# taaha-khan/2023-CompaCT-Image-Compression

Measured on AMD Instinct MI355X. Metric: MPixels/s encode+decode, 12-bit 512x512 CT batch, bytes-exact, higher is better.
Workload: dtype u16

## Files before the change

2023-compact-image-compression_amd/csrc/deflate_kernels.hip:

```cpp
#include <hip/hip_runtime.h>
#include <cstring>
#include <algorithm>

#include "cct_internal.h"
#include "../../include/compact_hip.h"

namespace cct {
namespace {

constexpr int MIN_MATCH = 3, MAX_MATCH = 258, WSIZE = 32768;
constexpr int MIN_LOOKAHEAD = MAX_MATCH + MIN_MATCH + 1;
constexpr int MAX_DIST = WSIZE - MIN_LOOKAHEAD;
constexpr int TOO_FAR = 4096;
constexpr int BLOCK_SYMS = 16383;
constexpr int BLOCK_SYMS_ML9 = 32767;
constexpr int L_CODES = 286, D_CODES = 30, BL_CODES = 19, HEAP_SIZE = 2 * L_CODES + 1;
constexpr int END_BLOCK = 256, MAX_BITS = 15, MAX_BL_BITS = 7;
constexpr uint32_t Z_FILTERED = 1, Z_HUFFMAN_ONLY = 2, Z_RLE = 3, Z_FIXED = 4;
__host__ __device__ __forceinline__ bool short_pass(uint32_t strategy) { return strategy == Z_HUFFMAN_ONLY || strategy == Z_RLE; }

__constant__ uint8_t c_extra_lbits[29] = {0,0,0,0,0,0,0,0,1,1,1,1,2,2,2,2,3,3,3,3,4,4,4,4,5,5,5,5,0};
__constant__ uint8_t c_extra_dbits[30] = {0,0,0,0,1,1,2,2,3,3,4,4,5,5,6,6,7,7,8,8,9,9,10,10,11,11,12,12,13,13};
__constant__ uint8_t c_extra_blbits[19] = {0,0,0,0,0,0,0,0,0,0,0,0,0,0,0,0,2,3,7};
__constant__ uint8_t c_bl_order[19] = {16,17,18,0,8,7,9,6,10,5,11,4,12,3,13,2,14,1,15};
__constant__ uint8_t c_length_code[256];
__constant__ uint16_t c_base_length[29];
__constant__ uint8_t c_dist_code[512];
__constant__ uint16_t c_base_dist[30];
__constant__ uint16_t c_static_lcode[288];
__constant__ uint8_t c_static_llen[288];
__constant__ uint16_t c_static_dcode[30];

template <int HB>
__device__ __forceinline__ uint32_t hash3(uint32_t b0, uint32_t b1, uint32_t b2)
{
	constexpr int SH = (HB + 2) / 3;
	return ((b0 << (2 * SH)) ^ (b1 << SH) ^ b2) & ((1u << HB) - 1u);
}

__device__ __forceinline__ int d_code(uint32_t dist) { return dist < 256 ? c_dist_code[dist] : c_dist_code[256 + (dist >> 7)]; }

struct MatchRec { uint16_t len_full, len_quarter, dist_full, dist_quarter; };
constexpr uint32_t GEN_MAX = 16383;
__device__ __forceinline__ uint2 pack_match(uint32_t len_full, uint32_t len_quarter, uint32_t dist_full, uint32_t dist_quarter, uint32_t gen)
{
	return make_uint2((len_full | ((gen & 127u) << 9)) | ((len_quarter | ((gen >> 7) << 9)) << 16), dist_full | (dist_quarter << 16));
}
__device__ __forceinline__ MatchRec checked_match(MatchRec r, uint32_t gen, uint32_t rw, uint32_t p, uint32_t L)
{
	const uint32_t tag = (uint32_t)(r.len_full >> 9) | ((uint32_t)(r.len_quarter >> 9) << 7);
	const uint32_t lookahead = L - min(p, L);
	const uint32_t max_len = lookahead < (uint32_t)MAX_MATCH ? lookahead : (uint32_t)MAX_MATCH;
	const bool maximal = (rw >> 15) && (rw & 0x7FFFu) >= max_len && p + 2 < L;
	MatchRec o;
	const bool ok = tag == gen;
// ... 58 lines not shown
#ifdef CCT_SORT_PROBE
	const bool compact = false;
#else
	const bool compact = HB == 15 && a.pos_mask != 0xFFFFFFFFu;
#endif
	const uint32_t dmax = (uint32_t)a.in_stride - 4u;
	auto fetch = [&](uint32_t tile_base, uint32_t (&ra)[E], uint32_t (&rb)[E]) {
		if (FIRST) {
#pragma unroll
			for (int d = 0; d < ND; d++) ra[d] = *reinterpret_cast<const uint32_t *>(in + min(tile_base + 256u * d + 4u * (uint32_t)lane, dmax));
			ra[ND] = *reinterpret_cast<const uint32_t *>(in + min(tile_base + 256u * ND, dmax));
#pragma unroll
			for (int e = 0; e < E; e++) rb[e] = compact ? a.run_len[base + min(tile_base + (uint32_t)(e * 64 + lane), last)] : 0u;
		} else {
#pragma unroll
			for (int e = 0; e < E; e++) {
				const uint64_t r = rec_src[min(tile_base + (uint32_t)(e * 64 + lane), last)];
				ra[e] = (uint32_t)r; rb[e] = (uint32_t)(r >> 32);
			}
		}
	};
	auto finish = [&](uint32_t tile_base, const uint32_t (&ra)[E], const uint32_t (&rb)[E], uint32_t (&h)[E], uint32_t (&p)[E]) {
#pragma unroll
		for (int e = 0; e < E; e++) {
			const uint32_t idx = tile_base + (uint32_t)(e * 64 + lane);
			if (FIRST) {
				const int la = (e & 3) * 16 + (lane >> 2);
				const uint32_t da = (uint32_t)__builtin_amdgcn_ds_bpermute(la << 2, (int)ra[e >> 2]);
				uint32_t db = (uint32_t)__builtin_amdgcn_ds_bpermute(((la + 1) & 63) << 2, (int)ra[e >> 2]);
				if ((e & 3) == 3) {
					const uint32_t nxt = (e >> 2) + 1 < ND ? (uint32_t)__builtin_amdgcn_readfirstlane((int)ra[(e >> 2) + 1 < ND ? (e >> 2) + 1 : 0]) : ra[ND];
					if (la == 63) db = nxt;
				}
				const uint32_t sh = (uint32_t)lane & 3u;
				const uint32_t w = __builtin_amdgcn_alignbyte(db, da, sh);
				const uint32_t b0 = w & 255u, b1 = (w >> 8) & 255u, b2 = (w >> 16) & 255u;
				h[e] = hash3<HB>(b0, b1, b2); p[e] = idx;
				if (compact) {
					const uint32_t b4 = (db >> (8u * sh)) & 255u;
					const uint32_t f16 = (b0 == b1 && b1 == b2) ? rb[e] : ((w >> 24) | (b4 << 8));
					h[e] |= (f16 << 15) | ((b0 >> 7) << 31); p[e] |= (b1 << 22) | (((b0 >> 5) & 3u) << 30);
				}
			}
			else { h[e] = rb[e]; p[e] = ra[e]; }
			if (idx >= npos) { h[e] = 0; p[e] = idx; }
		}
	};
	uint32_t hn[E], pn[E];
	{
		uint32_t ra[E], rb[E];
		fetch((uint32_t)(wave * 64 * E), ra, rb);
		finish((uint32_t)(wave * 64 * E), ra, rb, hn, pn);
	}
	for (uint32_t t0 = 0; t0 < npos; t0 += 1024 * E) {
		uint32_t h[E], p[E], rk[E], ra[E], rb[E];
		const uint32_t idx0 = t0 + (uint32_t)(wave * 64 * E + lane);
#pragma unroll
		for (int e = 0; e < E; e++) { h[e] = hn[e]; p[e] = pn[e]; }
		const uint32_t next_base = t0 + (uint32_t)(1024 * E + wave * 64 * E);
		fetch(next_base, ra, rb);
		for (int k = lane; k < NB; k += 64) wcnt[wave][k] = 0;
#pragma unroll
		for (int e = 0; e < E; e++) {
			const bool valid = idx0 + e * 64 < npos;
			const uint32_t d = FIRST ? (h[e] & 255u) : ((h[e] & HMASK) >> 8);
			uint64_t same = __ballot(valid);
#pragma unroll
			for (int b = 0; b < BITS; b++) {
				const bool bit = (d >> b) & 1u;
				const uint64_t bal = __ballot(bit);
				same &= bit ? bal : ~bal;
			}
			const uint32_t rank = (uint32_t)__popcll(same & lt_mask);
			uint32_t before = 0;
			if (valid) {
				before = wcnt[wave][d];
				if (rank == 0) wcnt[wave][d] = before + (uint32_t)__popcll(same);
			}
			rk[e] = before + rank;
		}
		lds_barrier();
		if (tid < NB) {
			uint32_t c[16], run = offs[tid];
#pragma unroll
			for (int w = 0; w < 16; w++) c[w] = wcnt[w][tid];
#pragma unroll
			for (int w = 0; w < 16; w++) { wcnt[w][tid] = run; run += c[w]; }
			offs[tid] = run;
		}
		lds_barrier();
#pragma unroll
		for (int e = 0; e < E; e++) asm volatile("" : "+v"(ra[e]), "+v"(rb[e]) :: "memory");
		finish(next_base, ra, rb, hn, pn);
#pragma unroll
		for (int e = 0; e < E; e++) {
			if (idx0 + e * 64 < npos) {
				const uint32_t d = FIRST ? (h[e] & 255u) : ((h[e] & HMASK) >> 8);
				const uint32_t dst = wcnt[wave][d] + rk[e];
				rec_dst[dst] = (uint64_t)p[e] | ((uint64_t)h[e] << 32);
			}
		}
	}
}

constexpr int LIGHT_STEPS = 12;

__device__ __forceinline__ bool xcd_slice(int n, int &s, uint32_t &part, uint32_t &nparts)
{
	const uint32_t lin = blockIdx.x + gridDim.x * blockIdx.y;
	const uint32_t c = lin & 7u, k = lin >> 3;
	nparts = gridDim.x;
	s = (int)(8u * (k / nparts) + c);
	part = k % nparts;
	return s < n;
}

__device__ __forceinline__ uint32_t nil_candidate(uint32_t p, uint32_t lookahead)
{
	return (lookahead < (uint32_t)MIN_LOOKAHEAD && p >= 32506u + 32768u && (p - 32506u) % 32768u == 0) ? p - 32506u : 0xFFFFFFFFu;
}

constexpr int RUNLEN_OUT = 2048 - 264;

template <bool SORT, int HB>
__global__ void __launch_bounds__(256) dfl_run_len_kernel(DeflateArgs a)
{
	constexpr int NH = 256 + (1 << (HB - 8));
	__shared__ uint32_t wtot[4];
	__shared__ uint32_t hist[SORT ? NH : 1];
	if (SORT) for (int t = threadIdx.x; t < NH; t += 256) hist[t] = 0;
	__syncthreads();
	const int s = blockIdx.y;
	const uint32_t L = a.in_sizes[s];
	const uint8_t *in = a.in + (size_t)s * a.in_stride;
	uint16_t *rl = a.run_len + (size_t)s * a.in_stride;
	const int lane = threadIdx.x & 63, wave = threadIdx.x >> 6;
	const uint32_t nchunks = (L + RUNLEN_OUT - 1) / RUNLEN_OUT;
	for (uint32_t c = blockIdx.x; c < nchunks; c += gridDim.x) {
		const uint32_t c0 = c * RUNLEN_OUT;
		const uint32_t g = c0 + threadIdx.x * 8;
		uint8_t b[12];
		if (g + 12 <= L && g >= 1) {
			uint64_t w;
			__builtin_memcpy(&w, in + g, 8);
#pragma unroll
			for (int k = 0; k < 8; k++) b[k + 1] = (uint8_t)(w >> (8 * k));
			b[0] = in[g - 1];
			uint32_t w2; __builtin_memcpy(&w2, in + g + 8, 4);
			b[9] = (uint8_t)w2; b[10] = (uint8_t)(w2 >> 8); b[11] = (uint8_t)(w2 >> 16);
		} else {
#pragma unroll
			for (int k = 0; k < 12; k++) { const int64_t y = (int64_t)g - 1 + k; b[k] = (y >= 0 && y < (int64_t)L) ? in[y] : 0; }
		}
		if (SORT) {
// ... 509 lines not shown
{
	len = 2; dist = 0;
	if (p >= npos || prev_len >= lazy) return;
	match_of(checked_match(mr[p], gen, rl[p], p, npos + 2), p, npos, prev_len, lazy, good, minl, len, dist);
}

__global__ void __launch_bounds__(256) dfl_rec_kernel(DeflateArgs a)
{
	const int s = blockIdx.y;
	const uint32_t L = a.in_sizes[s];
	const size_t base = (size_t)s * a.in_stride;
	const uint32_t npos = L >= MIN_MATCH ? L - 2 : 0;
	const MatchRec *mr = reinterpret_cast<const MatchRec *>(a.mr) + base;
	const uint16_t *rl = a.run_len + base;
	const uint32_t nblk64 = (L + 63) / 64;
	const int lane = threadIdx.x & 63;
	const uint32_t gen = *a.gen;
	const int lazy = (int)a.max_lazy, good = (int)a.good, minl = (int)a.min_len;
	const uint32_t lastp = npos ? npos - 1 : 0;
	const uint32_t wb_step = gridDim.x * (blockDim.x >> 6);
	struct Req { MatchRec m0, m1; uint32_t w0, w1; };
	auto request = [&](uint32_t wb) {
		const uint32_t p = wb * 64 + lane, pa = min(p, lastp), pb = min(p + 1, lastp);
		return Req{mr[pa], mr[pb], rl[pa], rl[pb]};
	};
	const uint32_t wb0 = blockIdx.x * (blockDim.x >> 6) + (threadIdx.x >> 6);
	Req nx = request(wb0);
	for (uint32_t wb = wb0; wb < nblk64; wb += wb_step) {
		const uint32_t p = wb * 64 + lane;
		const uint32_t blk_end = wb * 64 + 64;
		uint32_t rec = 0, nxt = blk_end, cnt = 0;
		const uint32_t pa = min(p, lastp), pb = min(p + 1, lastp);
		const Req cq = nx;
		nx = request(wb + wb_step);
		const MatchRec r0 = checked_match(cq.m0, gen, cq.w0, pa, L), r1 = checked_match(cq.m1, gen, cq.w1, pb, L);
		if (p < L) {
			int len, dist;
			match_of(r0, p, npos, 2, lazy, good, minl, len, dist);
			if (len < MIN_MATCH) { rec = 0; nxt = p + 1; cnt = 1; }
			else {
				uint32_t k = 0;
				for (;;) {
					int l2, d2;
					if (k == 0) match_of(r1, p + 1, npos, len, lazy, good, minl, l2, d2);
					else match_at(mr, rl, gen, p + k + 1, npos, len, lazy, good, minl, l2, d2);
					if (l2 > len) { len = l2; dist = d2; k++; } else break;
				}
				rec = k | ((uint32_t)len << 8) | ((uint32_t)dist << 17);
				nxt = p + k + (uint32_t)len;
				cnt = k + 1;
			}
		}
		a.rec32[base + p] = rec;
#pragma unroll
		for (int r = 0; r < 6; r++) {
			const bool inside = nxt < blk_end;
			const int j = inside ? (int)(nxt - wb * 64) : lane;
			const uint32_t n2 = __shfl(nxt, j), c2 = __shfl(cnt, j);
			if (inside) { nxt = n2; cnt += c2; }
		}
		a.exit_pos[base + p] = (nxt - blk_end) | (cnt << 16);
	}
}

__global__ void __launch_bounds__(256) dfl_rle_rec_kernel(DeflateArgs a)
{
	const int s = blockIdx.y;
	const uint32_t L = a.in_sizes[s];
	const size_t base = (size_t)s * a.in_stride;
	const uint16_t *rl = a.run_len + base;
	const uint32_t nblk64 = (L + 63) / 64;
	const int lane = threadIdx.x & 63;
	const uint32_t lastp = L ? L - 1 : 0;
	const uint32_t wb_step = gridDim.x * (blockDim.x >> 6);
	const uint32_t wb0 = blockIdx.x * (blockDim.x >> 6) + (threadIdx.x >> 6);
	uint32_t nx = rl[min(wb0 * 64 + lane, lastp)];
	for (uint32_t wb = wb0; wb < nblk64; wb += wb_step) {
		const uint32_t p = wb * 64 + lane;
		const uint32_t blk_end = wb * 64 + 64;
		const uint32_t rw = nx;
		nx = rl[min((wb + wb_step) * 64 + lane, lastp)];
		const uint32_t rw0 = (uint32_t)__shfl((int)rw, 0);
		const bool prev_eq = p >= 2 ? (rw >> 15) != 0 : (p == 1 && (rw0 & 0x7FFFu) >= 2u);
		const uint32_t run = rw & 0x7FFFu;
		uint32_t rec = 0, nxt = blk_end, cnt = 0;
		if (p < L) {
			const bool m = prev_eq && run >= (uint32_t)MIN_MATCH;
			rec = m ? (run << 8) | (1u << 17) : 0u;
			nxt = p + (m ? run : 1u);
			cnt = 1;
		}
		a.rec32[base + p] = rec;
#pragma unroll
		for (int r = 0; r < 6; r++) {
			const bool inside = nxt < blk_end;
			const int j = inside ? (int)(nxt - wb * 64) : lane;
			const uint32_t n2 = __shfl(nxt, j), c2 = __shfl(cnt, j);
			if (inside) { nxt = n2; cnt += c2; }
		}
		a.exit_pos[base + p] = (nxt - blk_end) | (cnt << 16);
	}
}

template <uint32_t BS>
__global__ void __launch_bounds__(256) dfl_huff_symbols_kernel(DeflateArgs a)
{
	const int s = blockIdx.y;
	const uint32_t L = a.in_sizes[s];
	const size_t base = (size_t)s * a.in_stride;
	const uint32_t *in4 = reinterpret_cast<const uint32_t *>(a.in + base);
	uint4 *sym4 = reinterpret_cast<uint4 *>(a.sym + base);
	uint32_t *bend = a.blk_end + (size_t)s * a.max_blocks, *btop = a.blk_top + (size_t)s * a.max_blocks;
	if (blockIdx.x == 0 && threadIdx.x == 0) a.total_syms[s] = L;
	const uint32_t nq = (L + 3) / 4;
	for (uint32_t q = blockIdx.x * blockDim.x + threadIdx.x; q < nq; q += gridDim.x * blockDim.x) {
		const uint32_t w = in4[q], p0 = 4 * q;
		uint32_t v[4];
#pragma unroll
		for (int k = 0; k < 4; k++) {
			const uint32_t p = p0 + (uint32_t)k;
			v[k] = p < L ? (w >> (8 * k)) & 255u : 0u;
			if (p < L && p % BS == BS - 1) { bend[p / BS] = p + 1; btop[p / BS] = p; }
		}
		sym4[q] = make_uint4(v[0], v[1], v[2], v[3]);
	}
}

#ifndef CCT_WALK_T
#define CCT_WALK_T 256
#endif
constexpr int WALK_T = CCT_WALK_T;
__global__ void __launch_bounds__(WALK_T) dfl_walk_kernel(DeflateArgs a, int n)
{
	__shared__ uint32_t s_land[WALK_T];
	__shared__ uint32_t s_wsum[WALK_T / 64];
	const int s = blockIdx.x;
	(void)n;
	const uint32_t L = a.in_sizes[s];
	const size_t base = (size_t)s * a.in_stride;
	const size_t bbase = (size_t)s * (a.in_stride / 64);
	const uint32_t *exit_rec = a.exit_pos + base;
	const int tid = threadIdx.x, lane = tid & 63, wave = tid >> 6;
	const uint32_t seg = (((L + WALK_T - 1) / WALK_T) + 63) & ~63u;
	const uint32_t seg_end = min(L, (uint32_t)(tid + 1) * seg);
	uint32_t start = min(L, (uint32_t)tid * seg), land = start, cnt = 0;
// ... 646 lines not shown
	for (int q = 0; q < nb; q++) {
		TreeScratch &S = S4[q];
		BlockTables *bt = a.block_tables + ((size_t)s * a.max_blocks + m0 + q);
		for (int i = lane; i < L_CODES; i += 64) { bt->lcode[i] = S.code[i]; bt->llen[i] = (uint8_t)S.len[i]; }
		if (lane < D_CODES) { bt->dcode[lane] = S.dcode[lane]; bt->dlen[lane] = (uint8_t)S.dlen[lane]; }
	}
}

__global__ void __launch_bounds__(256) dfl_adler_kernel(DeflateArgs a)
{
	__shared__ unsigned long long sa[256], sb[256];
	const int s = blockIdx.x;
	const uint32_t L = a.in_sizes[s];
	const uint8_t *in = a.in + (size_t)s * a.in_stride;
	unsigned long long A = 0, B = 0;
	const uint32_t nfull = L / 16;
	constexpr int U = 8;
	for (uint32_t g0 = threadIdx.x; g0 < nfull; g0 += blockDim.x * U) {
		uint4 v[U];
#pragma unroll
		for (int u = 0; u < U; u++) v[u] = *reinterpret_cast<const uint4 *>(in + (size_t)min(g0 + (uint32_t)u * blockDim.x, nfull - 1) * 16);
#pragma unroll
		for (int u = 0; u < U; u++) {
			const uint32_t g = g0 + (uint32_t)u * blockDim.x;
			if (g >= nfull) continue;
			const uint32_t w[4] = {v[u].x, v[u].y, v[u].z, v[u].w};
			uint32_t sd = 0, sk = 0;
#pragma unroll
			for (int k = 0; k < 16; k++) { const uint32_t d = (w[k >> 2] >> ((k & 3) * 8)) & 0xFFu; sd += d; sk += (uint32_t)k * d; }
			A += sd;
			B += (unsigned long long)(L - g * 16) * sd - sk;
		}
	}
	if (threadIdx.x == 0)
		for (uint32_t i = nfull * 16; i < L; i++) { const unsigned long long d = in[i]; A += d; B += (unsigned long long)(L - i) * d; }
	sa[threadIdx.x] = A; sb[threadIdx.x] = B;
	__syncthreads();
	for (int st = 128; st > 0; st >>= 1) {
		if ((int)threadIdx.x < st) { sa[threadIdx.x] += sa[threadIdx.x + st]; sb[threadIdx.x] += sb[threadIdx.x + st]; }
		__syncthreads();
	}
	if (threadIdx.x == 0) {
		const uint32_t lo = (uint32_t)((1ull + sa[0]) % 65521ull);
		const uint32_t hi = (uint32_t)(((unsigned long long)L + sb[0]) % 65521ull);
		a.adler[s] = (hi << 16) | lo;
	}
}

__global__ void dfl_layout_kernel(DeflateArgs a, int n)
{
	const int s = blockIdx.x * blockDim.x + threadIdx.x;
	if (s >= n) return;
	uint8_t *out = a.out + (size_t)s * a.out_stride;
	for (int i = 0; i < 13; i++) out[i] = a.header13[i];
	out[13] = 0x78; out[14] = (uint8_t)a.zlib_flg;
	uint64_t bit = 8ull * 15;
	BlockMeta *meta = a.block_meta + (size_t)s * a.max_blocks;
	const uint32_t nb = a.n_blocks[s];
	for (uint32_t m = 0; m < nb; m++) {
		BlockMeta bm = meta[m];
		bm.bit_off = bit;
		if (bm.type == 0) {
			bit = (bit + 3 + 7) & ~7ull;
			bit += 32 + 8ull * bm.stored_len;
		} else {
			bit += 3 + bm.hdr_nbits + bm.body_bits;
		}
		if (bm.last) bit = (bit + 7) & ~7ull;
		meta[m] = bm;
	}
	const uint64_t byte = bit >> 3;
	const uint32_t ad = a.adler[s];
	out[byte + 0] = (uint8_t)(ad >> 24); out[byte + 1] = (uint8_t)(ad >> 16);
	out[byte + 2] = (uint8_t)(ad >> 8);  out[byte + 3] = (uint8_t)ad;
	a.out_sizes[s] = (uint32_t)(byte + 4);
}

__device__ __forceinline__ void or_bits(uint32_t *words, uint64_t bit, uint64_t value, int nbits)
{
	if (nbits == 0) return;
	const uint64_t w = bit >> 5;
	const int sh = (int)(bit & 31);
	const uint64_t lo = value << sh;
	const uint64_t hi = sh ? (value >> (64 - sh)) : 0ull;
	atomicOr(&words[w], (uint32_t)lo);
	if (sh + nbits > 32) atomicOr(&words[w + 1], (uint32_t)(lo >> 32));
	if (sh + nbits > 64) atomicOr(&words[w + 2], (uint32_t)hi);
}

__global__ void __launch_bounds__(256) dfl_emit_kernel(DeflateArgs a)
{
	__shared__ uint32_t wsum[4];
	__shared__ unsigned long long s_run;
	const int s = blockIdx.y, m = blockIdx.x;
	if ((uint32_t)m >= a.n_blocks[s]) return;
	const BlockMeta bm = a.block_meta[(size_t)s * a.max_blocks + m];
	const BlockTables *bt = a.block_tables + ((size_t)s * a.max_blocks + m);
	uint8_t *out = a.out + (size_t)s * a.out_stride;
	uint32_t *words = reinterpret_cast<uint32_t *>(out);
	const uint8_t *in = a.in + (size_t)s * a.in_stride;
	uint64_t bit = bm.bit_off;
	if (bm.type == 0) {
		if (threadIdx.x == 0) or_bits(words, bit, (uint64_t)bm.last, 3);
		const uint64_t byte = ((bit + 3 + 7) & ~7ull) >> 3;
		if (threadIdx.x == 0) {
			out[byte] = (uint8_t)(bm.stored_len & 0xFF); out[byte + 1] = (uint8_t)(bm.stored_len >> 8);
			out[byte + 2] = (uint8_t)(~bm.stored_len & 0xFF); out[byte + 3] = (uint8_t)((~bm.stored_len >> 8) & 0xFF);
		}
		for (uint32_t i = threadIdx.x; i < bm.stored_len; i += blockDim.x) out[byte + 4 + i] = in[bm.in_begin + i];
		return;
	}
	if (threadIdx.x == 0) or_bits(words, bit, (uint64_t)((bm.type << 1) + bm.last), 3);
	bit += 3;
	if (bm.type == 2) {
		for (uint32_t i = threadIdx.x; i * 32 < bm.hdr_nbits; i += blockDim.x) {
			const int nb = (int)min(32u, bm.hdr_nbits - i * 32);
			or_bits(words, bit + 32ull * i, bt->hdr_bits[i], nb);
		}
		bit += bm.hdr_nbits;
	}
	const uint32_t *sym = a.sym + (size_t)s * a.in_stride + bm.first_sym;
	const bool dyn = bm.type == 2;
	const int lane = threadIdx.x & 63, wave = threadIdx.x >> 6;
	__shared__ uint16_t t_lcode[L_CODES + 2], t_dcode[D_CODES + 2];
	__shared__ uint8_t t_llen[L_CODES + 2], t_dlen[D_CODES + 2];
	__shared__ uint32_t wbuf[400];
	__shared__ uint8_t t_length_code[256], t_dist_code[512], t_extra_l[32], t_extra_d[32];
	__shared__ uint16_t t_base_length[32], t_base_dist[32];
	{
		const int t = threadIdx.x, t2 = min(t + 256, L_CODES - 1), td = min(t, D_CODES - 1), t29 = min(t, 28), t30 = min(t, 29);
		const uint16_t *lsrc = dyn ? bt->lcode : c_static_lcode, *dsrc = dyn ? bt->dcode : c_static_dcode;
		const uint8_t *llsrc = dyn ? bt->llen : c_static_llen;
		const uint16_t lc0 = lsrc[t], lc1 = lsrc[t2];
		const uint8_t ll0 = llsrc[t], ll1 = llsrc[t2];
		const uint16_t dc = dsrc[td];
		uint8_t dl = bt->dlen[td];
		if (!dyn) dl = 5;
		const uint8_t k0 = c_dist_code[t], k1 = c_dist_code[t + 256], lcd = c_length_code[t];
		const uint8_t xl = c_extra_lbits[t29], xd = c_extra_dbits[t30];
		const uint16_t bl = c_base_length[t29], bd = c_base_dist[t30];
		t_lcode[t] = lc0; t_llen[t] = ll0;
		if (t + 256 < L_CODES) { t_lcode[t + 256] = lc1; t_llen[t + 256] = ll1; }
		if (t < D_CODES) { t_dcode[t] = dc; t_dlen[t] = dl; }
		t_dist_code[t] = k0; t_dist_code[t + 256] = k1; t_length_code[t] = lcd;
		if (t < 29) { t_extra_l[t] = xl; t_base_length[t] = bl; }
		if (t < 30) { t_extra_d[t] = xd; t_base_dist[t] = bd; }
	}
	if (threadIdx.x == 0) s_run = bit;
	for (int i = threadIdx.x; i < 400; i += blockDim.x) wbuf[i] = 0;
	__syncthreads();
	const uint32_t last_sym = bm.nsym ? bm.nsym - 1 : 0;
	uint32_t vnext = sym[min((uint32_t)threadIdx.x, last_sym)];
	for (uint32_t base = 0; base <= bm.nsym; base += blockDim.x) {
		const uint32_t i = base + threadIdx.x;
		uint64_t bits = 0;
		int nb = 0;
		const uint32_t v = vnext;
		vnext = sym[min(i + blockDim.x, last_sym)];
		if (i < bm.nsym) {
			uint32_t dist = v >> 16;
			const uint32_t lc = v & 0xFFu;
			if (dist == 0) {
				bits = t_lcode[lc];
				nb = t_llen[lc];
			} else {
				int code = t_length_code[lc];
				const int lsym = code + 256 + 1;
				bits = t_lcode[lsym];
				nb = t_llen[lsym];
				int extra = t_extra_l[code];
				if (extra) { bits |= (uint64_t)(lc - t_base_length[code]) << nb; nb += extra; }
				dist--;
				code = dist < 256 ? t_dist_code[dist] : t_dist_code[256 + (dist >> 7)];
				bits |= (uint64_t)t_dcode[code] << nb;
				nb += t_dlen[code];
				extra = t_extra_d[code];
				if (extra) { bits |= (uint64_t)(dist - t_base_dist[code]) << nb; nb += extra; }
			}
		} else if (i == bm.nsym) {
			bits = t_lcode[END_BLOCK];
			nb = t_llen[END_BLOCK];
		}
		uint32_t inc = (uint32_t)nb;
#pragma unroll
		for (int d = 1; d < 64; d <<= 1) {
			const uint32_t t = __shfl_up(inc, d);
			if (lane >= d) inc += t;
		}
		if (lane == 63) wsum[wave] = inc;
		__syncthreads();
		uint32_t wb = 0, tot = 0;
		for (int w = 0; w < 4; w++) { if (w < wave) wb += wsum[w]; tot += wsum[w]; }
		const uint64_t run = s_run;
		const uint32_t lbit = (uint32_t)(run & 31) + wb + inc - (uint32_t)nb;
		if (nb) {
			const uint32_t w0 = lbit >> 5, sh = lbit & 31;
			const uint64_t lo = bits << sh;
			atomicOr(&wbuf[w0], (uint32_t)lo);
			if (sh + nb > 32) atomicOr(&wbuf[w0 + 1], (uint32_t)(lo >> 32));
			if (sh + nb > 64) atomicOr(&wbuf[w0 + 2], (uint32_t)(bits >> (64 - sh)));
		}
		__syncthreads();
		const uint32_t nwords = ((uint32_t)(run & 31) + tot + 31) >> 5;
		const uint64_t gw = run >> 5;
		for (uint32_t k = threadIdx.x; k < nwords; k += blockDim.x) {
			const uint32_t v = wbuf[k];
			if (v) atomicOr(&words[gw + k], v);
			wbuf[k] = 0;
		}
		if (threadIdx.x == 0) s_run = run + tot;
		__syncthreads();
	}
}

__global__ void __launch_bounds__(256) dfl_pack_offsets_kernel(const uint32_t *sizes, int n, uint64_t *offsets, int exact)
{
	if (threadIdx.x == 0 && blockIdx.x == 0) {
		uint64_t acc = 0;
		for (int i = 0; i < n; i++) { offsets[i] = acc; acc += exact ? sizes[i] : ((sizes[i] + 15u) & ~15u); }
		offsets[n] = acc;
	}
}
__global__ void __launch_bounds__(256) dfl_pack_kernel(const uint8_t *src, size_t stride, const uint32_t *sizes,
                                                       const uint64_t *offsets, uint8_t *dst)
{
	const int s = blockIdx.y;
	const uint32_t n16 = (sizes[s] + 15u) >> 4;
	const uint4 *in = reinterpret_cast<const uint4 *>(src + (size_t)s * stride);
	uint4 *out = reinterpret_cast<uint4 *>(dst + offsets[s]);
	for (uint32_t i = blockIdx.x * blockDim.x + threadIdx.x; i < n16; i += gridDim.x * blockDim.x) out[i] = in[i];
}

__global__ void dfl_offsets2_kernel(DeflateArgs a, int n)
{
	const size_t per = a.in_stride / 64;
	for (size_t i = blockIdx.x * (size_t)blockDim.x + threadIdx.x; i < (size_t)n * per; i += (size_t)gridDim.x * blockDim.x)
		a.blk_entry[i] = 0xFFFFFFFFu;
}

__global__ void dfl_offsets_kernel(DeflateArgs a, int n)
{
	if (blockIdx.x == 0) {
		for (int s = threadIdx.x; s < n; s += blockDim.x) { a.postloop_lit[s] = 0; a.heavy_count[s] = 0; a.deep_count[s] = 0; a.run_end_count[s] = 0; }
		if (threadIdx.x == 0) *a.gen = *a.gen % GEN_MAX + 1u;
	}
	const size_t nrc = (size_t)n * 2 * (size_t)a.run_chunks;
	for (size_t t = (size_t)blockIdx.x * blockDim.x + threadIdx.x; t < nrc; t += (size_t)gridDim.x * blockDim.x) a.run_counts[t] = 0;
}

}

bool deflate_level_args(int level, DeflateArgs &a)
{
	static const uint32_t T[6][5] = {
		{4, 4, 16, 16, 0x5E}, {8, 16, 32, 32, 0x5E}, {8, 16, 128, 128, 0x9C},
		{8, 32, 128, 256, 0xDA}, {32, 128, 258, 1024, 0xDA}, {32, 258, 258, 4096, 0xDA},
	};
	if (level < 4 || level > 9) return false;
	const uint32_t *t = T[level - 4];
	a.good = t[0]; a.max_lazy = t[1]; a.nice = t[2]; a.max_chain = t[3]; a.zlib_flg = t[4];
	return true;
}

bool deflate_strategy_args(int level, int strategy, DeflateArgs &a)
{
	if (strategy < 0 || strategy > (int)Z_FIXED) return false;
	a.strategy = (uint32_t)strategy;
	a.min_len = strategy == (int)Z_FILTERED ? 6u : (uint32_t)MIN_MATCH;
	if (short_pass((uint32_t)strategy)) {
		if (level < 1 || level > 9) return false;
		a.good = a.max_lazy = a.nice = a.max_chain = 0;
		a.zlib_flg = 0x01;
		return true;
	}
	if (!deflate_level_args(level, a)) return false;
	if (strategy == (int)Z_FIXED) a.zlib_flg = 0x01;
	return true;
}

bool deflate_mem_level_args(int mem_level, DeflateArgs &a)
{
	if (mem_level != 8 && mem_level != 9) return false;
	a.hash_bits = (uint32_t)mem_level + 7u;
	a.block_syms = (1u << (mem_level + 6)) - 1u;
	return true;
}

hipError_t deflate_init_tables()
{
	uint8_t length_code[256]; uint16_t base_length[29]; uint8_t dist_code[512]; uint16_t base_dist[30];
	uint16_t static_lcode[288]; uint8_t static_llen[288]; uint16_t static_dcode[30];
	static const int xl[29] = {0,0,0,0,0,0,0,0,1,1,1,1,2,2,2,2,3,3,3,3,4,4,4,4,5,5,5,5,0};
	static const int xd[30] = {0,0,0,0,1,1,2,2,3,3,4,4,5,5,6,6,7,7,8,8,9,9,10,10,11,11,12,12,13,13};
	int length = 0, code, n, dist = 0;
	for (code = 0; code < 28; code++) {
		base_length[code] = (uint16_t)length;
		for (n = 0; n < (1 << xl[code]); n++) length_code[length++] = (uint8_t)code;
	}
	length_code[length - 1] = (uint8_t)code;
	base_length[28] = 0;
	for (code = 0; code < 16; code++) {
		base_dist[code] = (uint16_t)dist;
		for (n = 0; n < (1 << xd[code]); n++) dist_code[dist++] = (uint8_t)code;
	}
	dist >>= 7;
	for (; code < 30; code++) {
		base_dist[code] = (uint16_t)(dist << 7);
		for (n = 0; n < (1 << (xd[code] - 7)); n++) dist_code[256 + dist++] = (uint8_t)code;
	}
	uint16_t bl_count[16] = {0}, next_code[16];
	n = 0;
	while (n <= 143) { static_llen[n++] = 8; bl_count[8]++; }
	while (n <= 255) { static_llen[n++] = 9; bl_count[9]++; }
	while (n <= 279) { static_llen[n++] = 7; bl_count[7]++; }
	while (n <= 287) { static_llen[n++] = 8; bl_count[8]++; }
	unsigned c = 0;
	for (int bits = 1; bits <= 15; bits++) { c = (c + bl_count[bits - 1]) << 1; next_code[bits] = (uint16_t)c; }
	auto rev = [](unsigned v, int len) { unsigned r = 0; do { r |= v & 1; v >>= 1; r <<= 1; } while (--len > 0); return r >> 1; };
	for (n = 0; n < 288; n++) static_lcode[n] = (uint16_t)rev(next_code[static_llen[n]]++, static_llen[n]);
	for (n = 0; n < 30; n++) static_dcode[n] = (uint16_t)rev((unsigned)n, 5);
	hipError_t e;
	if ((e = hipMemcpyToSymbol(HIP_SYMBOL(c_length_code), length_code, sizeof length_code)) != hipSuccess) return e;
	if ((e = hipMemcpyToSymbol(HIP_SYMBOL(c_base_length), base_length, sizeof base_length)) != hipSuccess) return e;
	if ((e = hipMemcpyToSymbol(HIP_SYMBOL(c_dist_code), dist_code, sizeof dist_code)) != hipSuccess) return e;
	if ((e = hipMemcpyToSymbol(HIP_SYMBOL(c_base_dist), base_dist, sizeof base_dist)) != hipSuccess) return e;
	if ((e = hipMemcpyToSymbol(HIP_SYMBOL(c_static_lcode), static_lcode, sizeof static_lcode)) != hipSuccess) return e;
	if ((e = hipMemcpyToSymbol(HIP_SYMBOL(c_static_llen), static_llen, sizeof static_llen)) != hipSuccess) return e;
	if ((e = hipMemcpyToSymbol(HIP_SYMBOL(c_static_dcode), static_dcode, sizeof static_dcode)) != hipSuccess) return e;
	return hipSuccess;
}

size_t deflate_sort_temp_bytes(size_t total, int n)
{
	(void)total; (void)n;
	return 0;
}

static hipError_t launch_deflate_short(const DeflateArgs &a, int n, hipStream_t st)
{
	const bool ml9 = a.block_syms == (uint32_t)BLOCK_SYMS_ML9;
	const int gx = (int)std::min<size_t>(64, (a.in_stride + 255) / 256);
	if (a.strategy == Z_RLE) {
		hipLaunchKernelGGL((dfl_run_len_kernel<false, 15>), dim3(gx, n), dim3(256), 0, st, a);
		hipLaunchKernelGGL(dfl_rle_rec_kernel, dim3(gx, n), dim3(256), 0, st, a);
		hipLaunchKernelGGL(dfl_offsets2_kernel, dim3(256), dim3(256), 0, st, a, n);
		hipLaunchKernelGGL(dfl_walk_kernel, dim3(n), dim3(WALK_T), 0, st, a, n);
		if (ml9) hipLaunchKernelGGL(dfl_symbols_kernel<BLOCK_SYMS_ML9>, dim3(gx, n), dim3(256), 0, st, a);
		else hipLaunchKernelGGL(dfl_symbols_kernel<BLOCK_SYMS>, dim3(gx, n), dim3(256), 0, st, a);
	} else {
		if (ml9) hipLaunchKernelGGL(dfl_huff_symbols_kernel<BLOCK_SYMS_ML9>, dim3(gx, n), dim3(256), 0, st, a);
		else hipLaunchKernelGGL(dfl_huff_symbols_kernel<BLOCK_SYMS>, dim3(gx, n), dim3(256), 0, st, a);
	}
	hipLaunchKernelGGL(dfl_adler_kernel, dim3(n), dim3(256), 0, st, a);
	hipLaunchKernelGGL(dfl_tree_kernel, dim3((a.max_blocks + TREE_BLOCKS - 1) / TREE_BLOCKS, n), dim3(64), 0, st, a);
	hipLaunchKernelGGL(dfl_layout_kernel, dim3((n + 63) / 64), dim3(64), 0, st, a, n);
	hipLaunchKernelGGL(dfl_emit_kernel, dim3(a.max_blocks, n), dim3(256), 0, st, a);
	return hipGetLastError();
}

hipError_t launch_deflate(const DeflateArgs &a, int n, void *sort_temp, size_t sort_temp_bytes, hipStream_t st, hipStream_t side,
                          const hipEvent_t *ev)
{
	hipError_t e;
	const bool ml9 = a.hash_bits == 16;
	if ((a.hash_bits != 15 && !ml9) || a.block_syms != (uint32_t)(ml9 ? BLOCK_SYMS_ML9 : BLOCK_SYMS)) return hipErrorInvalidValue;
	if (ml9 && a.pos_mask != 0xFFFFFFFFu) return hipErrorInvalidValue;
	if ((e = hipMemsetAsync(a.out, 0, (size_t)n * a.out_stride, st)) != hipSuccess) return e;
	if (short_pass(a.strategy)) return launch_deflate_short(a, n, st);
	if ((e = hipMemsetAsync(a.sort_hist, 0, (size_t)n * SORT_HIST * 4, st)) != hipSuccess) return e;
	hipLaunchKernelGGL(dfl_offsets_kernel, dim3(64), dim3(256), 0, st, a, n);
	const int gx = (int)std::min<size_t>(64, (a.in_stride + 255) / 256);
	(void)sort_temp; (void)sort_temp_bytes;
	if (ml9) {
		hipLaunchKernelGGL((dfl_run_len_kernel<true, 16>), dim3(gx, n), dim3(256), 0, st, a);
		hipLaunchKernelGGL((dfl_sort_pass_kernel<true, 16>), dim3(n), dim3(1024), 0, st, a);
		hipLaunchKernelGGL((dfl_sort_pass_kernel<false, 16>), dim3(n), dim3(1024), 0, st, a);
	} else {
		hipLaunchKernelGGL((dfl_run_len_kernel<true, 15>), dim3(gx, n), dim3(256), 0, st, a);
		hipLaunchKernelGGL((dfl_sort_pass_kernel<true, 15>), dim3(n), dim3(1024), 0, st, a);
		hipLaunchKernelGGL((dfl_sort_pass_kernel<false, 15>), dim3(n), dim3(1024), 0, st, a);
	}
	const bool fork = side != nullptr && ev != nullptr;
	hipStream_t s2 = fork ? side : st;
	if (fork) {
		if ((e = hipEventRecord(ev[0], st)) != hipSuccess) return e;
		if ((e = hipStreamWaitEvent(s2, ev[0], 0)) != hipSuccess) return e;
	}
	hipLaunchKernelGGL(dfl_run_lists_kernel, dim3(a.run_chunks, n), dim3(256), 0, s2, a);
	hipLaunchKernelGGL(dfl_run_info_kernel, dim3(8, n), dim3(256), 0, s2, a);
	const int gm_cap = a.pos_mask == COMPACT_POS_MASK ? 256 : 2048;
	const int gm = (int)std::min<size_t>(gm_cap, (a.in_stride + 255) / 256), n8 = (n + 7) & ~7;
	if (a.max_chain < 16 || a.max_chain > 4096 || a.nice < 16 || a.nice > (uint32_t)MAX_MATCH) return hipErrorInvalidValue;
	const bool ql = (a.max_chain >> 2) <= (uint32_t)LIGHT_STEPS;
	if (a.pos_mask == COMPACT_POS_MASK) {
		if (ql) hipLaunchKernelGGL((dfl_match_kernel<true, true>), dim3(gm, n8), dim3(256), 0, st, a, n);
		else hipLaunchKernelGGL((dfl_match_kernel<true, false>), dim3(gm, n8), dim3(256), 0, st, a, n);
	} else if (a.pos_mask == 0xFFFFFFFFu) {
		if (ql) hipLaunchKernelGGL((dfl_match_kernel<false, true>), dim3(gm, n8), dim3(256), 0, st, a, n);
		else hipLaunchKernelGGL((dfl_match_kernel<false, false>), dim3(gm, n8), dim3(256), 0, st, a, n);
	} else return hipErrorInvalidValue;
	if (fork) {
		if ((e = hipEventRecord(ev[1], st)) != hipSuccess) return e;
		if ((e = hipEventRecord(ev[2], s2)) != hipSuccess) return e;
		if ((e = hipStreamWaitEvent(s2, ev[1], 0)) != hipSuccess) return e;
		if ((e = hipStreamWaitEvent(st, ev[2], 0)) != hipSuccess) return e;
	}
	hipLaunchKernelGGL(dfl_match_heavy_kernel, dim3(gx, n8), dim3(256), 0, s2, a, n);
	hipLaunchKernelGGL(dfl_adler_kernel, dim3(n), dim3(256), 0, s2, a);
	hipLaunchKernelGGL(dfl_match_run_kernel, dim3(gx, n8), dim3(256), 0, st, a, n);
	if (fork) {
		if ((e = hipEventRecord(ev[3], s2)) != hipSuccess) return e;
		if ((e = hipStreamWaitEvent(st, ev[3], 0)) != hipSuccess) return e;
	}
	hipLaunchKernelGGL(dfl_rec_kernel, dim3(gx, n), dim3(256), 0, st, a);
	hipLaunchKernelGGL(dfl_offsets2_kernel, dim3(256), dim3(256), 0, st, a, n);
	hipLaunchKernelGGL(dfl_walk_kernel, dim3(n), dim3(WALK_T), 0, st, a, n);
	if (ml9) hipLaunchKernelGGL(dfl_symbols_kernel<BLOCK_SYMS_ML9>, dim3(gx, n), dim3(256), 0, st, a);
	else hipLaunchKernelGGL(dfl_symbols_kernel<BLOCK_SYMS>, dim3(gx, n), dim3(256), 0, st, a);
	hipLaunchKernelGGL(dfl_tree_kernel, dim3((a.max_blocks + TREE_BLOCKS - 1) / TREE_BLOCKS, n), dim3(64), 0, st, a);
	hipLaunchKernelGGL(dfl_layout_kernel, dim3((n + 63) / 64), dim3(64), 0, st, a, n);
	hipLaunchKernelGGL(dfl_emit_kernel, dim3(a.max_blocks, n), dim3(256), 0, st, a);
	return hipGetLastError();
}

__global__ void __launch_bounds__(256) dfl_pack_exact_kernel(const uint8_t *src, size_t stride, const uint32_t *sizes,
                                                             const uint64_t *offsets, uint8_t *dst)
{
	const int s = blockIdx.y;
	const uint32_t nbytes = sizes[s];
	const uint8_t *in = src + (size_t)s * stride;
	uint8_t *out = dst + offsets[s];
	for (uint32_t i = blockIdx.x * blockDim.x + threadIdx.x; i < nbytes; i += gridDim.x * blockDim.x) out[i] = in[i];
}

hipError_t launch_pack(const uint8_t *src, size_t stride, const uint32_t *sizes, int n, uint64_t *offsets, uint8_t *dst,
                       int exact, hipStream_t st)
{
	hipLaunchKernelGGL(dfl_pack_offsets_kernel, dim3(1), dim3(64), 0, st, sizes, n, offsets, exact);
	if (exact) hipLaunchKernelGGL(dfl_pack_exact_kernel, dim3(32, n), dim3(256), 0, st, src, stride, sizes, offsets, dst);
	else hipLaunchKernelGGL(dfl_pack_kernel, dim3(16, n), dim3(256), 0, st, src, stride, sizes, offsets, dst);
	return hipGetLastError();
}

}
```

Baseline: 16220.

## Drop output and histogram memsets, fold blk_entry init, faster sort ranking and parallel pack offsets

Removes the full-output hipMemsetAsync by having emit write whole words directly, with atomics only on shared boundary words, and having the layout kernel zero boundary words and padding. The sort_hist memset and the offsets2 kernel are folded into existing kernels. The first radix pass gets a full-tile specialization and an mbcnt-based rank, and pack offsets become a 256-thread parallel scan. This cuts memset traffic and launches, but correctness now depends on every output byte being written exactly once or ORed safely.

```diff
diff --git a/2023-compact-image-compression_amd/csrc/deflate_kernels.hip b/2023-compact-image-compression_amd/csrc/deflate_kernels.hip
--- a/2023-compact-image-compression_amd/csrc/deflate_kernels.hip
+++ b/2023-compact-image-compression_amd/csrc/deflate_kernels.hip
@@ -1,6 +1,7 @@
 #include <hip/hip_runtime.h>
 #include <cstring>
 #include <algorithm>
+#include <type_traits>
 
 #include "cct_internal.h"
 #include "../../include/compact_hip.h"
@@ -165,7 +166,8 @@
 		fetch((uint32_t)(wave * 64 * E), ra, rb);
 		finish((uint32_t)(wave * 64 * E), ra, rb, hn, pn);
 	}
-	for (uint32_t t0 = 0; t0 < npos; t0 += 1024 * E) {
+	auto tile = [&](uint32_t t0, auto full_c) {
+		constexpr bool FULL = decltype(full_c)::value;
 		uint32_t h[E], p[E], rk[E], ra[E], rb[E];
 		const uint32_t idx0 = t0 + (uint32_t)(wave * 64 * E + lane);
 #pragma unroll
@@ -175,20 +177,36 @@
 		for (int k = lane; k < NB; k += 64) wcnt[wave][k] = 0;
 #pragma unroll
 		for (int e = 0; e < E; e++) {
-			const bool valid = idx0 + e * 64 < npos;
+			const bool valid = FULL || idx0 + e * 64 < npos;
 			const uint32_t d = FIRST ? (h[e] & 255u) : ((h[e] & HMASK) >> 8);
-			uint64_t same = __ballot(valid);
-#pragma unroll
-			for (int b = 0; b < BITS; b++) {
-				const bool bit = (d >> b) & 1u;
-				const uint64_t bal = __ballot(bit);
-				same &= bit ? bal : ~bal;
-			}
-			const uint32_t rank = (uint32_t)__popcll(same & lt_mask);
+			uint32_t slo, shi, rank;
+			if (FIRST) {
+				uint32_t dlo = 0, dhi = 0;
+#pragma unroll
+				for (int b = 0; b < BITS; b++) {
+					const uint32_t m = (uint32_t)__builtin_amdgcn_sbfe((int)d, (uint32_t)b, 1u);
+					const uint64_t bal = __ballot(m != 0u);
+					dlo |= (uint32_t)bal ^ m;
+					dhi |= (uint32_t)(bal >> 32) ^ m;
+				}
+				slo = ~dlo; shi = ~dhi;
+				if (!FULL) { const uint64_t bv = __ballot(valid); slo &= (uint32_t)bv; shi &= (uint32_t)(bv >> 32); }
+				rank = __builtin_amdgcn_mbcnt_hi(shi, __builtin_amdgcn_mbcnt_lo(slo, 0u));
+			} else {
+				uint64_t same = __ballot(valid);
+#pragma unroll
+				for (int b = 0; b < BITS; b++) {
+					const bool bit = (d >> b) & 1u;
+					const uint64_t bal = __ballot(bit);
+					same &= bit ? bal : ~bal;
+				}
+				rank = (uint32_t)__popcll(same & lt_mask);
+				slo = (uint32_t)same; shi = (uint32_t)(same >> 32);
+			}
 			uint32_t before = 0;
 			if (valid) {
 				before = wcnt[wave][d];
-				if (rank == 0) wcnt[wave][d] = before + (uint32_t)__popcll(same);
+				if (rank == 0) wcnt[wave][d] = before + (uint32_t)(__popc(slo) + __popc(shi));
 			}
 			rk[e] = before + rank;
 		}
@@ -207,12 +225,19 @@
 		finish(next_base, ra, rb, hn, pn);
 #pragma unroll
 		for (int e = 0; e < E; e++) {
-			if (idx0 + e * 64 < npos) {
+			if (FULL || idx0 + e * 64 < npos) {
 				const uint32_t d = FIRST ? (h[e] & 255u) : ((h[e] & HMASK) >> 8);
 				const uint32_t dst = wcnt[wave][d] + rk[e];
 				rec_dst[dst] = (uint64_t)p[e] | ((uint64_t)h[e] << 32);
 			}
 		}
+	};
+	uint32_t t0 = 0;
+	if (FIRST) {
+		for (; t0 + 1024u * E <= npos; t0 += 1024 * E) tile(t0, std::true_type{});
+		if (t0 < npos) tile(t0, std::false_type{});
+	} else {
+		for (; t0 < npos; t0 += 1024 * E) tile(t0, std::false_type{});
 	}
 }
 
@@ -828,6 +853,7 @@
 			}
 		}
 		a.rec32[base + p] = rec;
+		if (lane == 0) a.blk_entry[(size_t)s * (a.in_stride / 64) + wb] = 0xFFFFFFFFu;
 #pragma unroll
 		for (int r = 0; r < 6; r++) {
 			const bool inside = nxt < blk_end;
@@ -867,6 +893,7 @@
 			cnt = 1;
 		}
 		a.rec32[base + p] = rec;
+		if (lane == 0) a.blk_entry[(size_t)s * (a.in_stride / 64) + wb] = 0xFFFFFFFFu;
 #pragma unroll
 		for (int r = 0; r < 6; r++) {
 			const bool inside = nxt < blk_end;
@@ -1619,40 +1646,47 @@
 	const int s = blockIdx.x * blockDim.x + threadIdx.x;
 	if (s >= n) return;
 	uint8_t *out = a.out + (size_t)s * a.out_stride;
+	uint32_t *words = reinterpret_cast<uint32_t *>(out);
 	for (int i = 0; i < 13; i++) out[i] = a.header13[i];
 	out[13] = 0x78; out[14] = (uint8_t)a.zlib_flg;
+	out[15] = 0;
 	uint64_t bit = 8ull * 15;
+	uint64_t set_w = bit >> 5;
 	BlockMeta *meta = a.block_meta + (size_t)s * a.max_blocks;
 	const uint32_t nb = a.n_blocks[s];
 	for (uint32_t m = 0; m < nb; m++) {
-		BlockMeta bm = meta[m];
-		bm.bit_off = bit;
-		if (bm.type == 0) {
+		const uint32_t type = meta[m].type, last = meta[m].last, stored_len = meta[m].stored_len;
+		const uint32_t hdr_nbits = meta[m].hdr_nbits, body_bits = meta[m].body_bits;
+		meta[m].bit_off = bit;
+		if ((bit & 31) && (bit >> 5) != set_w) { set_w = bit >> 5; words[set_w] = 0; }
+		if (type == 0) {
 			bit = (bit + 3 + 7) & ~7ull;
-			bit += 32 + 8ull * bm.stored_len;
+			bit += 32 + 8ull * stored_len;
 		} else {
-			bit += 3 + bm.hdr_nbits + bm.body_bits;
-		}
-		if (bm.last) bit = (bit + 7) & ~7ull;
-		meta[m] = bm;
+			bit += 3 + hdr_nbits + body_bits;
+		}
+		if (last) {
+			if ((bit & 31) && (bit >> 5) != set_w) { set_w = bit >> 5; words[set_w] = 0; }
+			bit = (bit + 7) & ~7ull;
+		}
 	}
 	const uint64_t byte = bit >> 3;
 	const uint32_t ad = a.adler[s];
 	out[byte + 0] = (uint8_t)(ad >> 24); out[byte + 1] = (uint8_t)(ad >> 16);
 	out[byte + 2] = (uint8_t)(ad >> 8);  out[byte + 3] = (uint8_t)ad;
-	a.out_sizes[s] = (uint32_t)(byte + 4);
-}
-
-__device__ __forceinline__ void or_bits(uint32_t *words, uint64_t bit, uint64_t value, int nbits)
+	const uint64_t size = byte + 4, pad_end = min((size + 15) & ~15ull, (uint64_t)a.out_stride);
+	for (uint64_t i = size; i < pad_end; i++) out[i] = 0;
+	a.out_sizes[s] = (uint32_t)size;
+}
+
+__device__ __forceinline__ void or_bits_lds(uint32_t *wbuf, uint32_t bit, uint64_t value, int nbits)
 {
 	if (nbits == 0) return;
-	const uint64_t w = bit >> 5;
-	const int sh = (int)(bit & 31);
+	const uint32_t w = bit >> 5, sh = bit & 31;
 	const uint64_t lo = value << sh;
-	const uint64_t hi = sh ? (value >> (64 - sh)) : 0ull;
-	atomicOr(&words[w], (uint32_t)lo);
-	if (sh + nbits > 32) atomicOr(&words[w + 1], (uint32_t)(lo >> 32));
-	if (sh + nbits > 64) atomicOr(&words[w + 2], (uint32_t)hi);
+	atomicOr(&wbuf[w], (uint32_t)lo);
+	if (sh + nbits > 32) atomicOr(&wbuf[w + 1], (uint32_t)(lo >> 32));
+	if (sh + nbits > 64) atomicOr(&wbuf[w + 2], (uint32_t)(value >> (64 - sh)));
 }
 
 __global__ void __launch_bounds__(256) dfl_emit_kernel(DeflateArgs a)
@@ -1666,25 +1700,23 @@
 	uint8_t *out = a.out + (size_t)s * a.out_stride;
 	uint32_t *words = reinterpret_cast<uint32_t *>(out);
 	const uint8_t *in = a.in + (size_t)s * a.in_stride;
-	uint64_t bit = bm.bit_off;
+	const uint64_t bit0 = bm.bit_off;
 	if (bm.type == 0) {
-		if (threadIdx.x == 0) or_bits(words, bit, (uint64_t)bm.last, 3);
-		const uint64_t byte = ((bit + 3 + 7) & ~7ull) >> 3;
+		const uint64_t hb = bit0 >> 3, byte = ((bit0 + 3 + 7) & ~7ull) >> 3, end = byte + 4 + bm.stored_len;
+		const uint64_t w_first = (bit0 & 31) ? bit0 >> 5 : ~0ull, w_last = (end & 3) ? end >> 2 : ~0ull;
+		auto put = [&](uint64_t i, uint32_t v) {
+			const uint64_t w = i >> 2;
+			if (w == w_first || w == w_last) { if (v) atomicOr(&words[w], v << (8 * (uint32_t)(i & 3))); }
+			else out[i] = (uint8_t)v;
+		};
 		if (threadIdx.x == 0) {
-			out[byte] = (uint8_t)(bm.stored_len & 0xFF); out[byte + 1] = (uint8_t)(bm.stored_len >> 8);
-			out[byte + 2] = (uint8_t)(~bm.stored_len & 0xFF); out[byte + 3] = (uint8_t)((~bm.stored_len >> 8) & 0xFF);
-		}
-		for (uint32_t i = threadIdx.x; i < bm.stored_len; i += blockDim.x) out[byte + 4 + i] = in[bm.in_begin + i];
+			put(hb, (uint32_t)bm.last << (bit0 & 7));
+			if (byte - 1 > hb) put(byte - 1, 0);
+			put(byte, bm.stored_len & 0xFF); put(byte + 1, (bm.stored_len >> 8) & 0xFF);
+			put(byte + 2, ~bm.stored_len & 0xFF); put(byte + 3, (~bm.stored_len >> 8) & 0xFF);
+		}
+		for (uint32_t i = threadIdx.x; i < bm.stored_len; i += blockDim.x) put(byte + 4 + i, in[bm.in_begin + i]);
 		return;
-	}
-	if (threadIdx.x == 0) or_bits(words, bit, (uint64_t)((bm.type << 1) + bm.last), 3);
-	bit += 3;
-	if (bm.type == 2) {
-		for (uint32_t i = threadIdx.x; i * 32 < bm.hdr_nbits; i += blockDim.x) {
-			const int nb = (int)min(32u, bm.hdr_nbits - i * 32);
-			or_bits(words, bit + 32ull * i, bt->hdr_bits[i], nb);
-		}
-		bit += bm.hdr_nbits;
 	}
 	const uint32_t *sym = a.sym + (size_t)s * a.in_stride + bm.first_sym;
 	const bool dyn = bm.type == 2;
@@ -1713,9 +1745,36 @@
 		if (t < 29) { t_extra_l[t] = xl; t_base_length[t] = bl; }
 		if (t < 30) { t_extra_d[t] = xd; t_base_dist[t] = bd; }
 	}
-	if (threadIdx.x == 0) s_run = bit;
 	for (int i = threadIdx.x; i < 400; i += blockDim.x) wbuf[i] = 0;
 	__syncthreads();
+	const uint64_t first_w = bit0 >> 5;
+	const bool first_shared = (bit0 & 31) != 0;
+	auto flush = [&](uint64_t run, uint32_t tot) {
+		const uint32_t nfull = ((uint32_t)(run & 31) + tot) >> 5;
+		const uint64_t gw = run >> 5;
+		for (uint32_t k = threadIdx.x; k < nfull; k += blockDim.x) {
+			const uint32_t v = wbuf[k];
+			if (k == 0 && first_shared && gw == first_w) atomicOr(&words[gw], v);
+			else words[gw + k] = v;
+			if (k) wbuf[k] = 0;
+		}
+		if (threadIdx.x == 0) {
+			const uint32_t carry = wbuf[nfull];
+			if (nfull) wbuf[nfull] = 0;
+			wbuf[0] = carry;
+			s_run = run + tot;
+		}
+	};
+	{
+		const uint32_t r31 = (uint32_t)(bit0 & 31);
+		if (threadIdx.x == 0) or_bits_lds(wbuf, r31, (uint64_t)((bm.type << 1) + bm.last), 3);
+		if (dyn)
+			for (uint32_t i = threadIdx.x; i * 32 < bm.hdr_nbits; i += blockDim.x)
+				or_bits_lds(wbuf, r31 + 3 + 32 * i, bt->hdr_bits[i], (int)min(32u, bm.hdr_nbits - i * 32));
+		__syncthreads();
+		flush(bit0, 3 + (dyn ? bm.hdr_nbits : 0u));
+		__syncthreads();
+	}
 	const uint32_t last_sym = bm.nsym ? bm.nsym - 1 : 0;
 	uint32_t vnext = sym[min((uint32_t)threadIdx.x, last_sym)];
 	for (uint32_t base = 0; base <= bm.nsym; base += blockDim.x) {
@@ -1768,25 +1827,34 @@
 			if (sh + nb > 64) atomicOr(&wbuf[w0 + 2], (uint32_t)(bits >> (64 - sh)));
 		}
 		__syncthreads();
-		const uint32_t nwords = ((uint32_t)(run & 31) + tot + 31) >> 5;
-		const uint64_t gw = run >> 5;
-		for (uint32_t k = threadIdx.x; k < nwords; k += blockDim.x) {
-			const uint32_t v = wbuf[k];
-			if (v) atomicOr(&words[gw + k], v);
-			wbuf[k] = 0;
-		}
-		if (threadIdx.x == 0) s_run = run + tot;
-		__syncthreads();
+		flush(run, tot);
+		__syncthreads();
+	}
+	if (threadIdx.x == 0) {
+		const uint64_t end = s_run;
+		if (end & 31) atomicOr(&words[end >> 5], wbuf[0]);
 	}
 }
 
 __global__ void __launch_bounds__(256) dfl_pack_offsets_kernel(const uint32_t *sizes, int n, uint64_t *offsets, int exact)
 {
-	if (threadIdx.x == 0 && blockIdx.x == 0) {
-		uint64_t acc = 0;
-		for (int i = 0; i < n; i++) { offsets[i] = acc; acc += exact ? sizes[i] : ((sizes[i] + 15u) & ~15u); }
-		offsets[n] = acc;
-	}
+	__shared__ unsigned long long part[256];
+	if (blockIdx.x != 0) return;
+	const int t = threadIdx.x, per = (n + 255) / 256, i0 = min(t * per, n), i1 = min(i0 + per, n);
+	auto sz = [&](int i) -> uint64_t { return exact ? sizes[i] : ((sizes[i] + 15u) & ~15u); };
+	uint64_t sum = 0;
+	for (int i = i0; i < i1; i++) sum += sz(i);
+	part[t] = sum;
+	__syncthreads();
+	for (int d = 1; d < 256; d <<= 1) {
+		const uint64_t o = t >= d ? part[t - d] : 0ull;
+		__syncthreads();
+		part[t] += o;
+		__syncthreads();
+	}
+	uint64_t acc = part[t] - sum;
+	for (int i = i0; i < i1; i++) { offsets[i] = acc; acc += sz(i); }
+	if (t == 255) offsets[n] = part[255];
 }
 __global__ void __launch_bounds__(256) dfl_pack_kernel(const uint8_t *src, size_t stride, const uint32_t *sizes,
                                                        const uint64_t *offsets, uint8_t *dst)
@@ -1798,13 +1866,6 @@
 	for (uint32_t i = blockIdx.x * blockDim.x + threadIdx.x; i < n16; i += gridDim.x * blockDim.x) out[i] = in[i];
 }
 
-__global__ void dfl_offsets2_kernel(DeflateArgs a, int n)
-{
-	const size_t per = a.in_stride / 64;
-	for (size_t i = blockIdx.x * (size_t)blockDim.x + threadIdx.x; i < (size_t)n * per; i += (size_t)gridDim.x * blockDim.x)
-		a.blk_entry[i] = 0xFFFFFFFFu;
-}
-
 __global__ void dfl_offsets_kernel(DeflateArgs a, int n)
 {
 	if (blockIdx.x == 0) {
@@ -1813,6 +1874,8 @@
 	}
 	const size_t nrc = (size_t)n * 2 * (size_t)a.run_chunks;
 	for (size_t t = (size_t)blockIdx.x * blockDim.x + threadIdx.x; t < nrc; t += (size_t)gridDim.x * blockDim.x) a.run_counts[t] = 0;
+	const size_t nsh = (size_t)n * SORT_HIST;
+	for (size_t t = (size_t)blockIdx.x * blockDim.x + threadIdx.x; t < nsh; t += (size_t)gridDim.x * blockDim.x) a.sort_hist[t] = 0;
 }
 
 }
@@ -1910,7 +1973,6 @@
 	if (a.strategy == Z_RLE) {
 		hipLaunchKernelGGL((dfl_run_len_kernel<false, 15>), dim3(gx, n), dim3(256), 0, st, a);
 		hipLaunchKernelGGL(dfl_rle_rec_kernel, dim3(gx, n), dim3(256), 0, st, a);
-		hipLaunchKernelGGL(dfl_offsets2_kernel, dim3(256), dim3(256), 0, st, a, n);
 		hipLaunchKernelGGL(dfl_walk_kernel, dim3(n), dim3(WALK_T), 0, st, a, n);
 		if (ml9) hipLaunchKernelGGL(dfl_symbols_kernel<BLOCK_SYMS_ML9>, dim3(gx, n), dim3(256), 0, st, a);
 		else hipLaunchKernelGGL(dfl_symbols_kernel<BLOCK_SYMS>, dim3(gx, n), dim3(256), 0, st, a);
@@ -1932,9 +1994,7 @@
 	const bool ml9 = a.hash_bits == 16;
 	if ((a.hash_bits != 15 && !ml9) || a.block_syms != (uint32_t)(ml9 ? BLOCK_SYMS_ML9 : BLOCK_SYMS)) return hipErrorInvalidValue;
 	if (ml9 && a.pos_mask != 0xFFFFFFFFu) return hipErrorInvalidValue;
-	if ((e = hipMemsetAsync(a.out, 0, (size_t)n * a.out_stride, st)) != hipSuccess) return e;
 	if (short_pass(a.strategy)) return launch_deflate_short(a, n, st);
-	if ((e = hipMemsetAsync(a.sort_hist, 0, (size_t)n * SORT_HIST * 4, st)) != hipSuccess) return e;
 	hipLaunchKernelGGL(dfl_offsets_kernel, dim3(64), dim3(256), 0, st, a, n);
 	const int gx = (int)std::min<size_t>(64, (a.in_stride + 255) / 256);
 	(void)sort_temp; (void)sort_temp_bytes;
@@ -1980,7 +2040,6 @@
 		if ((e = hipStreamWaitEvent(st, ev[3], 0)) != hipSuccess) return e;
 	}
 	hipLaunchKernelGGL(dfl_rec_kernel, dim3(gx, n), dim3(256), 0, st, a);
-	hipLaunchKernelGGL(dfl_offsets2_kernel, dim3(256), dim3(256), 0, st, a, n);
 	hipLaunchKernelGGL(dfl_walk_kernel, dim3(n), dim3(WALK_T), 0, st, a, n);
 	if (ml9) hipLaunchKernelGGL(dfl_symbols_kernel<BLOCK_SYMS_ML9>, dim3(gx, n), dim3(256), 0, st, a);
 	else hipLaunchKernelGGL(dfl_symbols_kernel<BLOCK_SYMS>, dim3(gx, n), dim3(256), 0, st, a);
@@ -2003,7 +2062,7 @@
 hipError_t launch_pack(const uint8_t *src, size_t stride, const uint32_t *sizes, int n, uint64_t *offsets, uint8_t *dst,
                        int exact, hipStream_t st)
 {
-	hipLaunchKernelGGL(dfl_pack_offsets_kernel, dim3(1), dim3(64), 0, st, sizes, n, offsets, exact);
+	hipLaunchKernelGGL(dfl_pack_offsets_kernel, dim3(1), dim3(256), 0, st, sizes, n, offsets, exact);
 	if (exact) hipLaunchKernelGGL(dfl_pack_exact_kernel, dim3(32, n), dim3(256), 0, st, src, stride, sizes, offsets, dst);
 	else hipLaunchKernelGGL(dfl_pack_kernel, dim3(16, n), dim3(256), 0, st, src, stride, sizes, offsets, dst);
 	return hipGetLastError();
```

Result: no change. 16230 (median of 2 runs) (+0.1%).
